# kaddly/GraphNeuralNetwork

Measured on NVIDIA B200. Metric: aggregated_edges_per_sec, higher is better.
Workload: dtype f32

## Files before the change

graphneuralnetwork_b200/_lib.py:

```python
from __future__ import annotations

import ctypes as C
import os
from pathlib import Path

_PKG = Path(__file__).resolve().parent
LIB_PATH = _PKG / "libgnn_b200.so"

i32, i64, f32, f64, u64 = C.c_int32, C.c_int64, C.c_float, C.c_double, C.c_uint64
ptr, size_t, cint = C.c_void_p, C.c_size_t, C.c_int

SIGNATURES = {
    "gnn_version": (cint, []),
    "gnn_last_error_string": (C.c_char_p, []),
    "gnn_status_string": (C.c_char_p, [cint]),
    "gnn_launch_count": (i64, []),
    "gnn_set_tuning": (cint, [C.c_char_p, cint]),
    "gnn_get_tuning": (cint, [C.c_char_p, C.POINTER(cint)]),
    "gnn_build_csr_from_coo_workspace_size": (size_t, [i64, i64]),
    "gnn_build_csr_from_coo": (cint, [ptr, ptr, ptr, i64, i64, i64, ptr, ptr, ptr, ptr, ptr, size_t, ptr]),
    "gnn_dense_mask_count_workspace_size": (size_t, [i64]),
    "gnn_dense_mask_count": (cint, [ptr, cint, i64, i64, i64, ptr, ptr, size_t, ptr]),
    "gnn_dense_mask_fill": (cint, [ptr, cint, i64, i64, i64, ptr, ptr, ptr]),
    "gnn_csr_transpose_workspace_size": (size_t, [i64, i64, i64]),
# ... 6 lines not shown
    "gnn_spmm_csr_planned_f32": (cint, [ptr, ptr, ptr, ptr, ptr, i64, i64, i32, i64, i64, ptr, i64, i64, ptr, i64, i32,
                                        cint, i32, ptr, i32, ptr, size_t, ptr]),
    "gnn_spmm_csr_planned_bf16": (cint, [ptr, ptr, ptr, ptr, ptr, i64, i64, i32, i64, i64, ptr, i64, i64, ptr, i64, i32,
                                         cint, i32, ptr, i32, ptr, size_t, ptr]),
    "gnn_sddmm_coo_f32": (cint, [ptr, ptr, cint, i64, ptr, i64, ptr, i64, i32, ptr, ptr]),
    "gnn_semantic_workspace_size": (i64, [i32]),
    "gnn_semantic_scores_f32": (cint, [ptr, i64, ptr, ptr, i64, i32, i32, ptr, ptr, ptr, i64, ptr]),
    "gnn_semantic_combine_f32": (cint, [ptr, ptr, i64, i32, i32, ptr, ptr]),
    "gnn_semantic_combine_bwd_f32": (cint, [ptr, ptr, ptr, i64, i32, i32, ptr, ptr, ptr, i64, ptr]),
    "gnn_semantic_scores_bwd_f32": (cint, [ptr, i64, ptr, ptr, ptr, i64, i32, i32, ptr, i64, ptr, ptr, ptr, i64, ptr]),
    "gnn_gather_reduce_f32": (cint, [ptr, i64, i64, ptr, cint, i64, i32, i32, cint, ptr, i64, ptr, ptr]),
    "gnn_gather_reduce_bf16": (cint, [ptr, i64, i64, ptr, cint, i64, i32, i32, cint, ptr, i64, ptr, ptr]),
    "gnn_gather_reduce_multi_f32": (cint, [ptr, i64, i64, i32, cint, i32, ptr, cint, ptr, ptr, ptr, ptr, ptr]),
    "gnn_gather_reduce_multi_bf16": (cint, [ptr, i64, i64, i32, cint, i32, ptr, cint, ptr, ptr, ptr, ptr, ptr]),
    "gnn_gather_reduce_multi_f32_split": (cint, [ptr, i64, i64, i32, cint, i32, ptr, cint, ptr, ptr, ptr, ptr, ptr, ptr]),
    "gnn_gather_reduce_typed_f32": (cint, [ptr, i64, i64, i32, ptr, cint, i64, i32, i32, cint, ptr, i64, ptr]),
    "gnn_gather_reduce_bwd_f32": (cint, [ptr, ptr, i64, i32, f32, ptr, i64, ptr, i64, i32, ptr]),
    "gnn_gather_reduce_bwd_dense_f32": (cint, [ptr, i64, ptr, i64, i32, i32, f32, ptr, ptr]),
    "gnn_sample_neighbors": (cint, [ptr, ptr, ptr, cint, i64, i32, u64, ptr, ptr, cint, ptr]),
    "gnn_gat_scores_f32": (cint, [ptr, i64, ptr, ptr, i64, i32, i32, ptr, ptr, ptr]),
    "gnn_gat_fused_fwd_f32": (cint, [ptr, ptr, ptr, i64, ptr, ptr, i64, i64, i32, i32, f32, cint, cint, ptr, ptr, ptr,
                                     i64, ptr, ptr, ptr, i64, i64, i64, ptr]),
    "gnn_gat_fused_bwd_f32": (cint, [ptr, ptr, ptr, ptr, ptr, ptr, i64, ptr, ptr, ptr, ptr, ptr, ptr, i64, i64, i32,
                                     i32, f32, cint, ptr, ptr, i64, ptr, ptr, ptr, i64, ptr, i64, ptr, i64, i64, cint,
                                     ptr, ptr, i64, ptr]),
    "gnn_gat_fused_fwd_train_f32": (cint, [ptr, ptr, ptr, i64, ptr, ptr, i64, i64, i32, i32, f32, cint, cint, ptr, ptr,
                                           ptr, ptr, ptr, i64, ptr, ptr, ptr, i64, i64, i64, ptr]),
    "gnn_gat_fused_fwd_train_bf16": (cint, [ptr, ptr, ptr, i64, ptr, ptr, i64, i64, i32, i32, f32, cint, cint, ptr, ptr,
                                            ptr, ptr, ptr, i64, ptr, ptr, ptr, i64, i64, i64, ptr]),
    "gnn_gat_fused_fwd_bf16": (cint, [ptr, ptr, ptr, i64, ptr, ptr, i64, i64, i32, i32, f32, cint, cint, ptr, ptr, ptr,
# ... 17 lines not shown
    "gnn_spmm_csr_ex_f32": (cint, [ptr, ptr, ptr, ptr, ptr, i64, i64, i32, i64, i64, ptr, ptr]),
    "gnn_spmm_csr_ex_bf16": (cint, [ptr, ptr, ptr, ptr, ptr, i64, i64, i32, i64, i64, ptr, ptr]),
}



class SpmmOpts(C.Structure):
    _fields_ = [("struct_size", i32), ("accumulate", i32), ("accumulate_prefix", i64), ("rows_per_team", i32),
                ("relu", i32), ("bias", ptr), ("row_map", ptr), ("X2", ptr), ("ldx2", i64), ("split", i64),
                ("long_rows", ptr), ("n_long", i64), ("long_threshold", i64), ("chunk_off", ptr), ("n_chunks", i64),
                ("chunk_edges", i32), ("exclusion_smem_bytes", i32), ("workspace", ptr), ("workspace_bytes", size_t)]


class GatDropout(C.Structure):
    _fields_ = [("struct_size", i32), ("p", f32), ("seed", u64), ("seed_dev", ptr)]


class HaloOpts(C.Structure):
    _fields_ = [("struct_size", i32), ("mover", i32), ("ctas", i32), ("warps_per_cta", i32),
                ("claim_smem_bytes", i32), ("first_peer", i32)]


GNN_OK = 0
REDUCE = {"mean": 0, "sum": 1, "max": 2}
GAT_SOFTMAX, GAT_EXPNEG = 0, 1

_lib = None


class GnnError(RuntimeError):
# ... 42 lines not shown
```

graphneuralnetwork_b200/csrc/api.cu:

```cuda
#include "common.cuh"
#include <string.h>
#include <mutex>
#include <map>
#include <string>

namespace gnn {

static thread_local char t_err[512] = "";
std::atomic<int64_t> g_launches{0};

void set_error(const char* fmt, ...) {
  va_list ap;
  va_start(ap, fmt);
  vsnprintf(t_err, sizeof(t_err), fmt, ap);
  va_end(ap);
}

int num_sms() {
  static int cache[64] = {0};
  int dev = 0;
  if (cudaGetDevice(&dev) != cudaSuccess || dev < 0 || dev >= 64) return 148;
  if (cache[dev] == 0) {
    int n = 0;
    if (cudaDeviceGetAttribute(&n, cudaDevAttrMultiProcessorCount, dev) != cudaSuccess || n <= 0) n = 148;
    cache[dev] = n;
  }
  return cache[dev];
}

static std::mutex g_tune_mu;
static std::map<std::string, int>& tune_map() {
  static std::map<std::string, int> m = {
      {"sage.smem_kb", 48},
      {"sage.chunk_bytes", 12288},
      {"sage.force_ldg", 0},
      {"sage.ctas_per_sm", 4},
      {"sage.packed_add", -1},
      {"spmm.long_row", 2048},
      {"spmm.chunk", 8192},
      {"spmm.unroll", 0},
      {"spmm.ctas3", 1},
      {"spmm.rows_per_team", 0},
      {"spmm.team_edges", 512},
      {"gat.stage_edges", 128},
      {"gat.bwd_stage_edges", 64},
      {"gat.coop_min_avg_deg", 256},
      {"gat.long_row", 1024},
  };
  return m;
}
int tuning(const char* key, int dflt) {
// ... 56 lines not shown
```

graphneuralnetwork_b200/csrc/sage.cu:

```cuda
#include "rowreduce.cuh"

using namespace gnn;

namespace {

constexpr int kConsumerWarps = 5;
constexpr int kConsumerThreads = kConsumerWarps * 32;
constexpr int kSageThreads = 32 + kConsumerThreads;
constexpr int kMaxBlocks = 4;
constexpr int kIdDepth = 4;

template <typename T>
struct SageArgs {
  const T* table;
  int64_t ld;
  int32_t F;
  int32_t n_blocks;
  const int32_t* idx32[kMaxBlocks];
  const int64_t* idx64[kMaxBlocks];
  int64_t src_off[kMaxBlocks + 1];
  int32_t fanout[kMaxBlocks];
  int32_t kc[kMaxBlocks];
  float scale[kMaxBlocks];
  T* out[kMaxBlocks];
  int64_t ldo[kMaxBlocks];
  int32_t* argmax[kMaxBlocks];
  int32_t out_vec16[kMaxBlocks];
  int32_t row_bytes;
  int32_t stage_rows;
  int32_t stages;
  int32_t nvec;
  int64_t n_table_rows;
  int32_t split[kMaxBlocks];
  int64_t lo_off[kMaxBlocks];
};

__device__ __forceinline__ void add2(float& a0, float& a1, float x0, float x1) {
  asm("{\n\t.reg .b64 ra, rx;\n\tmov.b64 ra, {%0, %1};\n\tmov.b64 rx, {%2, %3};\n\t"
      "add.rn.f32x2 ra, ra, rx;\n\tmov.b64 {%0, %1}, ra;\n\t}"
      : "+f"(a0), "+f"(a1)
      : "f"(x0), "f"(x1));
}

template <typename T>
struct Vec16;
template <>
struct Vec16<float> {
  static constexpr int E = 4;
  static __device__ __forceinline__ void unpack(const uint4& w, float (&o)[4]) {
// ... 31 lines not shown
  if (g < a.src_off[a.n_blocks]) {
    int b = 0;
    while (b + 1 < a.n_blocks && g >= a.src_off[b + 1]) ++b;
    c.b = b;
    c.src = g - a.src_off[b];
    c.fan = a.fanout[b];
    c.kc = a.kc[b];
  }
}
template <typename T>
__device__ __forceinline__ void cursor_next(Cursor& c, const SageArgs<T>& a) {
  c.c0 += c.kc;
  if (c.c0 >= c.fan) cursor_set(c, a, c.g + gridDim.x);
}

template <typename T, int NV, int OP, bool PK = true>
__global__ void __launch_bounds__(kSageThreads) sage_tma_kernel(const SageArgs<T> a) {
  constexpr int E = Vec16<T>::E;
  extern __shared__ __align__(128) unsigned char smem[];
  const int S = a.stages;
  const int stage_bytes = a.stage_rows * a.row_bytes;
  uint64_t* full = reinterpret_cast<uint64_t*>(smem + (size_t)S * stage_bytes);
  uint64_t* empty = full + S;
  uint32_t* mask = reinterpret_cast<uint32_t*>(empty + S);

  const int warp = threadIdx.x >> 5;
  const int lane = threadIdx.x & 31;
  if (threadIdx.x == 0) {
    for (int i = 0; i < S; ++i) {
      mbar_init(full + i, 1);
      mbar_init(empty + i, kConsumerWarps);
// ... 62 lines not shown
          best[v][i] = 0;
        }
    };
    reset();
    Cursor cur;
    cursor_set(cur, a, blockIdx.x);
    int stage = 0;
    uint32_t par = 0;
    for (; cur.g < total_src; cursor_next(cur, a)) {
      const int c0 = cur.c0;
      const int rows = min(cur.kc, cur.fan - c0);
      mbar_wait(full + stage, par);
      const unsigned m = mask[stage];
      const unsigned char* sb = smem + (size_t)stage * stage_bytes;
      const unsigned all_rows = rows >= 32 ? 0xffffffffu : ((1u << rows) - 1u);
      if (OP != GNN_REDUCE_MAX && m == all_rows) {
#pragma unroll 5
        for (int k = 0; k < rows; ++k) {
#pragma unroll
          for (int v = 0; v < NV; ++v) {
            const int vi = t + v * kConsumerThreads;
            if (vi < a.nvec) {
              const uint4 w = *reinterpret_cast<const uint4*>(sb + (size_t)k * a.row_bytes + (size_t)vi * 16);
              if (PK) {
                Vec16<T>::add(w, acc[v]);
              } else {
                float x[E];
                Vec16<T>::unpack(w, x);
#pragma unroll
                for (int i = 0; i < E; ++i) acc[v][i] += x[i];
              }
            }
          }
        }
      } else {
#pragma unroll 4
        for (int k = 0; k < rows; ++k) {
          if (!((m >> k) & 1u)) continue;
#pragma unroll
          for (int v = 0; v < NV; ++v) {
            const int vi = t + v * kConsumerThreads;
            if (vi < a.nvec) {
              const uint4 w = *reinterpret_cast<const uint4*>(sb + (size_t)k * a.row_bytes + (size_t)vi * 16);
              float x[E];
              Vec16<T>::unpack(w, x);
#pragma unroll
              for (int i = 0; i < E; ++i) {
                if (OP == GNN_REDUCE_MAX) {
                  if (x[i] > acc[v][i]) {
                    acc[v][i] = x[i];
                    best[v][i] = c0 + k;
                  }
                } else {
                  acc[v][i] += x[i];
                }
              }
            }
          }
        }
      }
// ... 49 lines not shown
              for (int i = 0; i < E; ++i)
                if (col0 + i < a.F) a.argmax[b][cur.src * a.ldo[b] + col0 + i] = best[v][i];
            }
          }
        }
        reset();
      }
      if (++stage == S) {
        stage = 0;
        par ^= 1u;
      }
    }
  }
}

template <typename T, int NV, int OP, bool PK>
int launch_tma_pk(const SageArgs<T>& a, size_t smem_bytes, int grid, cudaStream_t st) {
  static size_t configured[64] = {};
  int dev = 0;
  const bool cached = cudaGetDevice(&dev) == cudaSuccess && dev >= 0 && dev < 64;
  if (!cached || smem_bytes > configured[dev]) {
    GNN_CUDA(cudaFuncSetAttribute(sage_tma_kernel<T, NV, OP, PK>, cudaFuncAttributeMaxDynamicSharedMemorySize,
                                  (int)smem_bytes));
    if (cached) configured[dev] = smem_bytes;
  }
  sage_tma_kernel<T, NV, OP, PK><<<grid, kSageThreads, smem_bytes, st>>>(a);
  GNN_LAUNCH_CHECK();
  return GNN_OK;
}

template <typename T, int NV, int OP>
int launch_tma_inst(const SageArgs<T>& a, size_t smem_bytes, int grid, cudaStream_t st) {
  const int knob = tuning("sage.packed_add", -1);
  const bool pk = (OP != GNN_REDUCE_MAX) && (knob < 0 ? sizeof(T) == 2 : knob != 0);
  if (pk) return launch_tma_pk<T, NV, OP, true>(a, smem_bytes, grid, st);
  return launch_tma_pk<T, NV, OP, false>(a, smem_bytes, grid, st);
}

template <typename T, int OP>
int launch_tma(const SageArgs<T>& a, size_t smem_bytes, int grid, cudaStream_t st) {
  const int nv = (a.nvec + kConsumerThreads - 1) / kConsumerThreads;
  switch (nv) {
    case 1: return launch_tma_inst<T, 1, OP>(a, smem_bytes, grid, st);
    case 2: return launch_tma_inst<T, 2, OP>(a, smem_bytes, grid, st);
    case 3: return launch_tma_inst<T, 3, OP>(a, smem_bytes, grid, st);
    case 4: return launch_tma_inst<T, 4, OP>(a, smem_bytes, grid, st);
    default: break;
  }
  set_error("TMA gather: row too wide (nvec=%d)", a.nvec);
  return GNN_ERR_UNSUPPORTED;
}

template <typename T>
struct GatherBlock {
  const void* idx;
  int idx_bits;
  int64_t n_src;
  int32_t fanout;
  T* out;
  int64_t ldo;
  int32_t* argmax;
  int32_t split = 0;
  int64_t lo_off = 0;
};

template <typename T>
int gather_reduce_impl(const T* table, int64_t ld, int64_t n_table_rows, int32_t F, int reduce,
                       const GatherBlock<T>* blocks, int n_blocks, cudaStream_t st) {
  GNN_REQUIRE(F >= 0 && n_blocks >= 0 && n_blocks <= kMaxBlocks, GNN_ERR_BAD_ARG, "bad size (F=%d, blocks=%d, max %d)",
              F, n_blocks, kMaxBlocks);
  GNN_REQUIRE(reduce == GNN_REDUCE_MEAN || reduce == GNN_REDUCE_SUM || reduce == GNN_REDUCE_MAX, GNN_ERR_BAD_ARG,
              "unknown reduce %d (GraphSAGE_Pytorch/models/Aggregator.py:26 raises ValueError)", reduce);
  GNN_REQUIRE(n_table_rows < 0x7fffffffLL, GNN_ERR_UNSUPPORTED, "table rows do not fit int32");
  int64_t total_src = 0;
  for (int b = 0; b < n_blocks; ++b) {
    const GatherBlock<T>& k = blocks[b];
    GNN_REQUIRE(k.n_src >= 0 && k.fanout >= 0, GNN_ERR_BAD_ARG, "negative size");
    if (k.n_src == 0 || F == 0) continue;
    GNN_REQUIRE(k.fanout > 0, GNN_ERR_BAD_ARG, "fanout must be positive");
    GNN_REQUIRE(table && k.out, GNN_ERR_BAD_ARG, "null table/out");
    GNN_REQUIRE(k.idx == nullptr || k.idx_bits == 32 || k.idx_bits == 64, GNN_ERR_BAD_ARG, "idx_bits must be 32 or 64");
    GNN_REQUIRE(ld >= F && k.ldo >= F, GNN_ERR_BAD_ARG, "leading dimension smaller than F");
    GNN_REQUIRE(!k.split || (sizeof(T) == 4 && reduce != GNN_REDUCE_MAX && k.lo_off >= F && k.ldo % 4 == 0 &&
                             k.lo_off % 4 == 0 && aligned_to(k.out, 8)),
                GNN_ERR_BAD_ARG, "hi/lo fp16 output needs an fp32 table, mean/sum, 8-byte aligned planes");
    GNN_REQUIRE(k.idx != nullptr || k.n_src * (int64_t)k.fanout <= n_table_rows, GNN_ERR_BAD_ARG,
                "identity block needs n_src*fanout <= n_table_rows");
    total_src += k.n_src;
  }
  if (total_src == 0 || F == 0) return GNN_OK;

  const int esz = (int)sizeof(T);
  const int row_bytes = (int)round_up((size_t)F * esz, 16);
  const bool tma_ok = !tuning("sage.force_ldg", 0) && aligned_to(table, 16) && ((ld * esz) % 16 == 0) &&
                      (int64_t)row_bytes <= ld * esz && row_bytes >= 256 && (row_bytes / 16) <= 4 * kConsumerThreads;
  if (tma_ok) {
    SageArgs<T> a{};
    a.table = table;
    a.ld = ld;
    a.F = F;
    a.n_table_rows = n_table_rows;
    a.row_bytes = row_bytes;
    a.nvec = row_bytes / 16;
    const int E = 16 / esz;
    int kc0 = tuning("sage.chunk_bytes", 12288) / row_bytes;
    kc0 = kc0 < 1 ? 1 : kc0;
    kc0 = kc0 > 32 ? 32 : kc0;
    const size_t budget = (size_t)tuning("sage.smem_kb", 48) * 1024;
// ... 6 lines not shown
      a.idx32[nb] = (k.idx && k.idx_bits == 32) ? (const int32_t*)k.idx : nullptr;
      a.idx64[nb] = (k.idx && k.idx_bits == 64) ? (const int64_t*)k.idx : nullptr;
      a.fanout[nb] = k.fanout;
      int kc = kc0 > k.fanout ? k.fanout : kc0;
      const int nchunk = (k.fanout + kc - 1) / kc;
      kc = (k.fanout + nchunk - 1) / nchunk;
      a.kc[nb] = kc;
      stage_rows = kc > stage_rows ? kc : stage_rows;
      a.scale[nb] = (reduce == GNN_REDUCE_MEAN) ? 1.0f / (float)k.fanout : 1.0f;
      a.out[nb] = k.out;
      a.ldo[nb] = k.ldo;
      a.argmax[nb] = (reduce == GNN_REDUCE_MAX) ? k.argmax : nullptr;
      a.out_vec16[nb] = aligned_to(k.out, 16) && ((k.ldo * esz) % 16 == 0) && ((int64_t)a.nvec * E <= k.ldo);
      a.split[nb] = k.split;
      a.lo_off[nb] = k.lo_off;
      a.src_off[nb + 1] = a.src_off[nb] + k.n_src;
      ++nb;
    }
    a.n_blocks = nb;
    a.stage_rows = stage_rows;
    int stages = (int)(budget / ((size_t)stage_rows * row_bytes));
    stages = stages > 8 ? 8 : stages;
    GNN_REQUIRE(stages >= 2, GNN_ERR_UNSUPPORTED, "row of %d bytes does not fit the shared-memory ring", row_bytes);
    a.stages = stages;
    const size_t smem_bytes = (size_t)stages * stage_rows * row_bytes + (size_t)stages * (16 + 4) + 16;
    int64_t grid = (int64_t)num_sms() * tuning("sage.ctas_per_sm", 4);
    grid = grid > total_src ? total_src : grid;
    switch (reduce) {
      case GNN_REDUCE_MAX: return launch_tma<T, GNN_REDUCE_MAX>(a, smem_bytes, (int)grid, st);
      default: return launch_tma<T, GNN_REDUCE_SUM>(a, smem_bytes, (int)grid, st);
// ... 11 lines not shown
    r.fanout = k.fanout;
    r.col32 = (k.idx && k.idx_bits == 32) ? (const int32_t*)k.idx : nullptr;
    r.col64 = (k.idx && k.idx_bits == 64) ? (const int64_t*)k.idx : nullptr;
    r.val = nullptr;
    r.src_div = 0;
    r.scale = (reduce == GNN_REDUCE_MEAN) ? 1.0f / (float)k.fanout : 1.0f;
    r.n_src_rows = (int32_t)n_table_rows;
    r.X = table;
    r.ldx = ld;
    r.Y = k.out;
    r.ldy = k.ldo;
    r.n_rows = k.n_src;
    r.F = F;
    r.skip_deg_gt = 0;
    r.argmax = (reduce == GNN_REDUCE_MAX) ? k.argmax : nullptr;
    const int rc = (reduce == GNN_REDUCE_MAX) ? launch_row_reduce<T, 1>(r, st) : launch_row_reduce<T, 0>(r, st);
    if (rc != GNN_OK) return rc;
  }
  return GNN_OK;
}

template <typename T>
int gather_reduce_multi(const T* table, int64_t ld, int64_t n_table_rows, int32_t F, int reduce, int32_t n_blocks,
                        const void* const* idx, int idx_bits, const int64_t* n_src, const int32_t* fanout,
                        void* const* out, const int64_t* ld_out, cudaStream_t st) {
  GNN_REQUIRE(n_blocks >= 0 && n_blocks <= kMaxBlocks, GNN_ERR_UNSUPPORTED, "at most %d blocks per launch", kMaxBlocks);
  GNN_REQUIRE(n_blocks == 0 || (idx && n_src && fanout && out && ld_out), GNN_ERR_BAD_ARG, "null block array");
  GatherBlock<T> blocks[kMaxBlocks];
  for (int b = 0; b < n_blocks; ++b)
    blocks[b] = GatherBlock<T>{idx[b], idx_bits, n_src[b], fanout[b], (T*)out[b], ld_out[b], nullptr};
  return gather_reduce_impl<T>(table, ld, n_table_rows, F, reduce, blocks, n_blocks, st);
}
// ... 43 lines not shown
}

int gnn_gather_reduce_multi_f32_split(const float* table, int64_t ld_table, int64_t n_table_rows, int32_t F, int reduce,
                                      int32_t n_blocks, const void* const* idx_host, int idx_bits,
                                      const int64_t* n_src_host, const int32_t* fanout_host, void* const* out_hi_host,
                                      const int64_t* ld_out_host, const int64_t* lo_off_host, gnn_stream_t stream) {
  GNN_REQUIRE(n_blocks >= 0 && n_blocks <= kMaxBlocks, GNN_ERR_UNSUPPORTED, "at most %d blocks per launch", kMaxBlocks);
  GNN_REQUIRE(n_blocks == 0 || (idx_host && n_src_host && fanout_host && out_hi_host && ld_out_host && lo_off_host),
              GNN_ERR_BAD_ARG, "null block array");
  GatherBlock<float> blocks[kMaxBlocks];
  for (int b = 0; b < n_blocks; ++b) {
    blocks[b] = GatherBlock<float>{idx_host[b], idx_bits, n_src_host[b], fanout_host[b], (float*)out_hi_host[b],
                                   ld_out_host[b], nullptr};
    blocks[b].split = 1;
    blocks[b].lo_off = lo_off_host[b];
  }
  return gather_reduce_impl<float>(table, ld_table, n_table_rows, F, reduce, blocks, n_blocks, (cudaStream_t)stream);
}

int gnn_gather_reduce_multi_bf16(const void* table, int64_t ld_table, int64_t n_table_rows, int32_t F, int reduce,
                                 int32_t n_blocks, const void* const* idx_host, int idx_bits,
                                 const int64_t* n_src_host, const int32_t* fanout_host, void* const* out_host,
                                 const int64_t* ld_out_host, gnn_stream_t stream) {
  return gather_reduce_multi<__nv_bfloat16>((const __nv_bfloat16*)table, ld_table, n_table_rows, F, reduce, n_blocks,
                                            idx_host, idx_bits, n_src_host, fanout_host, out_host, ld_out_host,
                                            (cudaStream_t)stream);
}

int gnn_gather_reduce_typed_f32(const float* table, int64_t ld_row, int64_t n_nodes, int32_t n_types, const void* idx,
                                int idx_bits, int64_t n_src, int32_t fanout, int32_t F, int reduce, float* out,
// ... 74 lines not shown
```

graphneuralnetwork_b200/functional.py:

```python
from __future__ import annotations

from typing import Optional

import torch

from . import _lib
from .graph import CSRGraph, _p, _require_cuda, _stream_ptr, index_block_transpose


def _rowmajor(x: torch.Tensor) -> torch.Tensor:
    if x.dim() != 2:
        raise _lib.GnnError(f"expected a 2-D feature matrix, got shape {tuple(x.shape)}")
    if x.stride(1) != 1 and x.shape[1] > 1:
        x = x.contiguous()
    if x.shape[0] > 1 and x.stride(0) < x.shape[1]:
        x = x.contiguous()
    return x


def _ld(x: torch.Tensor) -> int:
    return x.stride(0) if x.shape[0] > 1 else max(x.shape[1], 1)


def _padded_empty(rows: int, F: int, dtype, device) -> torch.Tensor:
# ... 258 lines not shown
        if idx.numel() != n_src * fanout:
            raise _lib.GnnError(f"index block has {idx.numel()} ids, expected n_src*fanout = {n_src * fanout}")
        idxs.append(idx)
    for o in outs_hi:
        if o.dtype != torch.float16 or o.stride(1) != 1:
            raise _lib.GnnError("gather_reduce_multi_split: outputs must be fp16 views with unit column stride")
    idx_arr = (C.c_void_p * nb)(*[_p(i) for i in idxs])
    nsrc_arr = (C.c_int64 * nb)(*[int(b[1]) for b in blocks])
    fan_arr = (C.c_int32 * nb)(*[int(b[2]) for b in blocks])
    out_arr = (C.c_void_p * nb)(*[_p(o) for o in outs_hi])
    ldo_arr = (C.c_int64 * nb)(*[_ld(o) for o in outs_hi])
    lo_arr = (C.c_int64 * nb)(*[int(lo_off)] * nb)
    _lib.check(lib.gnn_gather_reduce_multi_f32_split(_p(table), _ld(table), N, F, _lib.REDUCE[reduce], nb, idx_arr,
                                                     bits or 64, nsrc_arr, fan_arr, out_arr, ldo_arr, lo_arr,
                                                     _stream_ptr()), "gnn_gather_reduce_multi_f32_split")


def sample_neighbors(g: CSRGraph, src: torch.Tensor, k: int, seed: int, out_dtype=torch.int32,
                     seed_offset: Optional[torch.Tensor] = None, out: Optional[torch.Tensor] = None) -> torch.Tensor:
    _require_cuda(src)
    lib = _lib.load()
    src = src.contiguous().view(-1)
    if src.dtype not in (torch.int32, torch.int64):
        src = src.to(torch.int64)
    if out is None:
        out = torch.empty(src.numel() * k, dtype=out_dtype, device=src.device)
    assert seed_offset is None or (seed_offset.dtype == torch.int64 and seed_offset.is_cuda)
    _lib.check(lib.gnn_sample_neighbors(_p(g.rowptr), _p(g.col), _p(src), 32 if src.dtype == torch.int32 else 64,
                                        src.numel(), int(k), int(seed) & 0xFFFFFFFFFFFFFFFF, _p(seed_offset), _p(out),
                                        32 if out.dtype == torch.int32 else 64, _stream_ptr()), "gnn_sample_neighbors")
# ... 433 lines not shown
```

graphneuralnetwork_b200/layers/sage.py:

```python
import torch
from torch import nn
import torch.nn.functional as F

from .. import _lib
from ..functional import gather_reduce, gather_reduce_multi_raw, gather_reduce_multi_split_raw, pad_table


class SampledBlock:

    def __init__(self, table: torch.Tensor, ids: torch.Tensor, fanout: int):
        self.table, self.ids, self.fanout = table, ids, int(fanout)
        self.n_src = ids.numel() // self.fanout


class NeighborAggregator(nn.Module):

    def __init__(self, input_dim, output_dim, use_bias=False, aggr_method="mean", **kwargs):
        super().__init__(**kwargs)
        self.input_dim, self.output_dim = input_dim, output_dim
        self.use_bias, self.aggr_method = use_bias, aggr_method
        self.weight = nn.Parameter(nn.init.xavier_uniform_(torch.empty(input_dim, output_dim)))
        if use_bias:
            self.bias = nn.Parameter(torch.zeros(output_dim))

# ... 100 lines not shown
        if getattr(self, "tensor_core_gemm", True) and layer0.aggr_neighbor_method in ("mean", "sum") \
                and table.stride(0) * 4 % 16 == 0 and F_in * 4 >= 256:
            try:
                return self._layer0_split_gemm(table, node_id_blocks, ld, n_hop, total)
            except _lib.GnnError:
                self.tensor_core_gemm = False
        key = (total, table.device)
        buf = getattr(self, "_l0_buf", None)
        if buf is None or buf[0] != key:
            Z = torch.zeros((total, 2 * ld), dtype=torch.float32, device=table.device)
            Wc = torch.zeros((2 * ld, H), dtype=torch.float32, device=table.device)
            self._l0_buf = buf = (key, Z, Wc)
        _, Z, Wc = buf
        Wc[:F_in].copy_(layer0.weight)
        Wc[ld:ld + F_in].copy_(layer0.aggregator.weight)
        blocks, outs, row = [], [], 0
        for hop in range(L):
            n = n_hop[hop]
            blocks += [(node_id_blocks[hop + 1], n, fan[hop]), (node_id_blocks[hop], n, 1)]
            outs += [Z[row:row + n, ld:ld + F_in], Z[row:row + n, :F_in]]
            row += n
        order = sorted(range(len(blocks)), key=lambda i: -blocks[i][1] * blocks[i][2])
        gather_reduce_multi_raw(table, [blocks[i] for i in order], layer0.aggr_neighbor_method,
                                outs=[outs[i] for i in order])
        hidden = torch.mm(Z, Wc)
        if layer0.activation:
            hidden = layer0.activation(hidden)
        out, row = [], 0
        for n in n_hop:
            out.append(hidden[row:row + n])
            row += n
        return out

    def _table_fits_fp16(self, table):
        key = (table.data_ptr(), table._version, tuple(table.shape))
        hit = getattr(self, "_fp16_ok", None)
        if hit is None or hit[0] != key:
            self._fp16_ok = hit = (key, bool((table.abs().max() < 3.0e4).item()))
        return hit[1]

    def _weight_planes(self, ld, device):
        layer0 = self.gcn[0]
        w, wa = layer0.weight, layer0.aggregator.weight
        F_in, H = layer0.input_dim, layer0.hidden_dim
        geom = (int(ld), torch.device(device))
        ver = (w._version, wa._version, w.data_ptr(), wa.data_ptr())
        planes = getattr(self, "_l0_planes", None)
# ... 13 lines not shown
            planes["ver"] = ver
        return planes["hi"], planes["lo"]

    def _layer0_split_gemm(self, table, node_id_blocks, ld, n_hop, total):
        if not self._table_fits_fp16(table):
            raise _lib.GnnError("table exceeds the fp16 range: fp32 product")
        L, fan, layer0 = self.num_layers, self.num_neighbors_list, self.gcn[0]
        F_in, H = layer0.input_dim, layer0.hidden_dim
        key = (total, table.device)
        buf = getattr(self, "_l0_split", None)
        if buf is None or buf[0] != key:
            Zs = torch.zeros((total, 4 * ld), dtype=torch.float16, device=table.device)
            self._l0_split = buf = (key, Zs)
        _, Zs = buf
        W_hi, W_lo = self._weight_planes(ld, table.device)
        blocks, outs, row = [], [], 0
        for hop in range(L):
            n = n_hop[hop]
            blocks += [(node_id_blocks[hop + 1], n, fan[hop]), (node_id_blocks[hop], n, 1)]
            outs += [Zs[row:row + n, ld:ld + F_in], Zs[row:row + n, :F_in]]
            row += n
        order = sorted(range(len(blocks)), key=lambda i: -blocks[i][1] * blocks[i][2])
        gather_reduce_multi_split_raw(table, [blocks[i] for i in order], layer0.aggr_neighbor_method,
                                      [outs[i] for i in order], lo_off=2 * ld)
        Z_hi, Z_lo = Zs[:, :2 * ld], Zs[:, 2 * ld:]
        hidden = torch.mm(Z_hi, W_hi, out_dtype=torch.float32)
        if getattr(self, "_addmm_out_dtype", True):
            try:
                hidden = torch.addmm(hidden, Z_lo, W_hi, out_dtype=torch.float32)
                hidden = torch.addmm(hidden, Z_hi, W_lo, out_dtype=torch.float32)
            except (RuntimeError, NotImplementedError):
                self._addmm_out_dtype = False
                hidden = torch.mm(Z_hi, W_hi, out_dtype=torch.float32)
        if not getattr(self, "_addmm_out_dtype", True):
            hidden += torch.mm(Z_lo, W_hi, out_dtype=torch.float32)
            hidden += torch.mm(Z_hi, W_lo, out_dtype=torch.float32)
        if layer0.activation:
            hidden = layer0.activation(hidden)
        out, row = [], 0
# ... 117 lines not shown
```

include/gnn_b200.h:

```cpp
#ifndef GNN_B200_H
#define GNN_B200_H

#include <stddef.h>
#include <stdint.h>

#ifdef __cplusplus
extern "C" {
#endif

typedef void* gnn_stream_t;

typedef enum {
  GNN_OK = 0,
  GNN_ERR_BAD_ARG = 1,
  GNN_ERR_MISALIGNED = 2,
  GNN_ERR_UNSUPPORTED = 3,
  GNN_ERR_CUDA = 4,
  GNN_ERR_WORKSPACE = 5
} gnn_status;

typedef enum { GNN_REDUCE_MEAN = 0, GNN_REDUCE_SUM = 1, GNN_REDUCE_MAX = 2 } gnn_reduce;

typedef enum {
  GNN_GAT_SOFTMAX = 0,
// ... 97 lines not shown
                           const void* idx, int idx_bits, int64_t n_src, int32_t fanout, int32_t F,
                           int reduce, void* out, int64_t ld_out, int32_t* argmax, gnn_stream_t stream);
int gnn_gather_reduce_multi_f32(const float* table, int64_t ld_table, int64_t n_table_rows, int32_t F, int reduce,
                                int32_t n_blocks, const void* const* idx_host, int idx_bits,
                                const int64_t* n_src_host, const int32_t* fanout_host,
                                void* const* out_host, const int64_t* ld_out_host, gnn_stream_t stream);
int gnn_gather_reduce_multi_bf16(const void* table, int64_t ld_table, int64_t n_table_rows, int32_t F, int reduce,
                                 int32_t n_blocks, const void* const* idx_host, int idx_bits,
                                 const int64_t* n_src_host, const int32_t* fanout_host,
                                 void* const* out_host, const int64_t* ld_out_host, gnn_stream_t stream);
int gnn_gather_reduce_multi_f32_split(const float* table, int64_t ld_table, int64_t n_table_rows, int32_t F, int reduce,
                                      int32_t n_blocks, const void* const* idx_host, int idx_bits,
                                      const int64_t* n_src_host, const int32_t* fanout_host,
                                      void* const* out_hi_host, const int64_t* ld_out_host,
                                      const int64_t* lo_off_host, gnn_stream_t stream);
int gnn_gather_reduce_typed_f32(const float* table, int64_t ld_row, int64_t n_nodes, int32_t n_types,
                                const void* idx, int idx_bits, int64_t n_src, int32_t fanout, int32_t F,
                                int reduce, float* out, int64_t ld_out, gnn_stream_t stream);
int gnn_gather_reduce_bwd_f32(const int64_t* rowptr_t, const int32_t* pos_t, int64_t n_table_rows,
                              int32_t fanout, float scale, const float* d_out, int64_t ld_dout,
                              float* d_table, int64_t ld_dtable, int32_t F, gnn_stream_t stream);
int gnn_gather_reduce_bwd_dense_f32(const float* d_out, int64_t ld_dout, const int32_t* argmax ,
                                    int64_t n_src, int32_t fanout, int32_t F, float scale,
                                    float* d_neigh , gnn_stream_t stream);

int gnn_sample_neighbors(const int64_t* rowptr, const int32_t* col, const void* src, int src_bits,
                         int64_t n_src, int32_t k, uint64_t seed, const int64_t* seed_offset_dev,
                         void* out, int out_bits, gnn_stream_t stream);

int gnn_gat_scores_f32(const float* Wh, int64_t ldw, const float* a_src, const float* a_dst,
// ... 131 lines not shown
```

Baseline: 2.022 billion.

## Echo gathered neighbor rows as next hop's self features; add narrow-row cp.async gather

In the layer-0 SAGE gather, the neighbor rows already staged for hop h are written out as the self-feature rows of hop h+1. This replaces the separate fanout-1 self gathers for all hops except the first, so those table rows are not read from global memory a second time. A separate cp.async warp-per-source kernel is added for fp32 mean/sum with rows of at most 512 bytes, used when split and echo are off. The echo path adds stores inside the TMA consumer loop and more template variants, and the narrow path bypasses the TMA pipeline for small F.

After: 2.062 billion, median of 6. 2.0% higher.

```diff
diff --git a/graphneuralnetwork_b200/_lib.py b/graphneuralnetwork_b200/_lib.py
--- a/graphneuralnetwork_b200/_lib.py
+++ b/graphneuralnetwork_b200/_lib.py
@@ -44,6 +44,7 @@
     "gnn_gather_reduce_multi_f32": (cint, [ptr, i64, i64, i32, cint, i32, ptr, cint, ptr, ptr, ptr, ptr, ptr]),
     "gnn_gather_reduce_multi_bf16": (cint, [ptr, i64, i64, i32, cint, i32, ptr, cint, ptr, ptr, ptr, ptr, ptr]),
     "gnn_gather_reduce_multi_f32_split": (cint, [ptr, i64, i64, i32, cint, i32, ptr, cint, ptr, ptr, ptr, ptr, ptr, ptr]),
+    "gnn_gather_reduce_multi_f32_ex": (cint, [ptr, i64, i64, i32, cint, i32, ptr, ptr]),
     "gnn_gather_reduce_typed_f32": (cint, [ptr, i64, i64, i32, ptr, cint, i64, i32, i32, cint, ptr, i64, ptr]),
     "gnn_gather_reduce_bwd_f32": (cint, [ptr, ptr, i64, i32, f32, ptr, i64, ptr, i64, i32, ptr]),
     "gnn_gather_reduce_bwd_dense_f32": (cint, [ptr, i64, ptr, i64, i32, i32, f32, ptr, ptr]),
@@ -91,6 +92,11 @@
 
 class GatDropout(C.Structure):
     _fields_ = [("struct_size", i32), ("p", f32), ("seed", u64), ("seed_dev", ptr)]
+
+
+class GatherBlock(C.Structure):
+    _fields_ = [("struct_size", i32), ("idx_bits", i32), ("idx", ptr), ("n_src", i64), ("fanout", i32), ("split", i32),
+                ("out", ptr), ("ld_out", i64), ("lo_off", i64), ("echo", ptr), ("ld_echo", i64)]
 
 
 class HaloOpts(C.Structure):
diff --git a/graphneuralnetwork_b200/csrc/api.cu b/graphneuralnetwork_b200/csrc/api.cu
--- a/graphneuralnetwork_b200/csrc/api.cu
+++ b/graphneuralnetwork_b200/csrc/api.cu
@@ -35,6 +35,7 @@
       {"sage.chunk_bytes", 12288},
       {"sage.force_ldg", 0},
       {"sage.ctas_per_sm", 4},
+      {"sage.narrow_ldg", -1},
       {"sage.packed_add", -1},
       {"spmm.long_row", 2048},
       {"spmm.chunk", 8192},
diff --git a/graphneuralnetwork_b200/csrc/sage.cu b/graphneuralnetwork_b200/csrc/sage.cu
--- a/graphneuralnetwork_b200/csrc/sage.cu
+++ b/graphneuralnetwork_b200/csrc/sage.cu
@@ -33,6 +33,9 @@
   int64_t n_table_rows;
   int32_t split[kMaxBlocks];
   int64_t lo_off[kMaxBlocks];
+  void* echo[kMaxBlocks];
+  int64_t ld_echo[kMaxBlocks];
+  int32_t echo_vec16[kMaxBlocks];
 };
 
 __device__ __forceinline__ void add2(float& a0, float& a1, float x0, float x1) {
@@ -94,7 +97,48 @@
   if (c.c0 >= c.fan) cursor_set(c, a, c.g + gridDim.x);
 }
 
-template <typename T, int NV, int OP, bool PK = true>
+template <typename T, int E>
+__device__ __forceinline__ void store_vec(void* out, int64_t ld, int64_t row, int col0, int F, int split,
+                                          int64_t lo_off, int vec16, const float (&o)[E]) {
+  if (sizeof(T) == 4 && split) {
+    __half* hrow = reinterpret_cast<__half*>(out) + row * ld + col0;
+    uint32_t hw[2], lw[2];
+#pragma unroll
+    for (int i = 0; i < 2; ++i) {
+      const __half h0 = __float2half_rn(o[2 * i]), h1 = __float2half_rn(o[2 * i + 1]);
+      const __half l0 = __float2half_rn(o[2 * i] - __half2float(h0));
+      const __half l1 = __float2half_rn(o[2 * i + 1] - __half2float(h1));
+      hw[i] = (uint32_t)__half_as_ushort(h0) | ((uint32_t)__half_as_ushort(h1) << 16);
+      lw[i] = (uint32_t)__half_as_ushort(l0) | ((uint32_t)__half_as_ushort(l1) << 16);
+    }
+    if (col0 + 3 < F) {
+      *reinterpret_cast<uint2*>(hrow) = make_uint2(hw[0], hw[1]);
+      *reinterpret_cast<uint2*>(hrow + lo_off) = make_uint2(lw[0], lw[1]);
+    } else {
+#pragma unroll
+      for (int i = 0; i < 4; ++i)
+        if (col0 + i < F) {
+          const __half h = __float2half_rn(o[i]);
+          hrow[i] = h;
+          hrow[lo_off + i] = __float2half_rn(o[i] - __half2float(h));
+        }
+    }
+  } else {
+    T* orow = reinterpret_cast<T*>(out) + row * ld + col0;
+    if (vec16) {
+      VecIO<T, E>::store(orow, o);
+    } else {
+#pragma unroll
+      for (int i = 0; i < E; ++i)
+        if (col0 + i < F) {
+          float o1[1] = {o[i]};
+          VecIO<T, 1>::store(orow + i, o1);
+        }
+    }
+  }
+}
+
+template <typename T, int NV, int OP, bool PK, bool ECHO>
 __global__ void __launch_bounds__(kSageThreads) sage_tma_kernel(const SageArgs<T> a) {
   constexpr int E = Vec16<T>::E;
   extern __shared__ __align__(128) unsigned char smem[];
@@ -187,6 +231,15 @@
       const unsigned m = mask[stage];
       const unsigned char* sb = smem + (size_t)stage * stage_bytes;
       const unsigned all_rows = rows >= 32 ? 0xffffffffu : ((1u << rows) - 1u);
+      void* const echo = ECHO ? a.echo[cur.b] : nullptr;
+      const int64_t erow0 = cur.src * cur.fan + c0;
+      auto echo_vec = [&](int k, int vi, const float (&x)[E]) {
+        float o[E];
+#pragma unroll
+        for (int i = 0; i < E; ++i) o[i] = x[i] + 0.f;
+        store_vec<T, E>(echo, a.ld_echo[cur.b], erow0 + k, vi * E, a.F, a.split[cur.b], a.lo_off[cur.b],
+                        a.echo_vec16[cur.b], o);
+      };
       if (OP != GNN_REDUCE_MAX && m == all_rows) {
 #pragma unroll 5
         for (int k = 0; k < rows; ++k) {
@@ -203,20 +256,32 @@
 #pragma unroll
                 for (int i = 0; i < E; ++i) acc[v][i] += x[i];
               }
+              if (ECHO && echo) {
+                float x[E];
+                Vec16<T>::unpack(w, x);
+                echo_vec(k, vi, x);
+              }
             }
           }
         }
       } else {
 #pragma unroll 4
         for (int k = 0; k < rows; ++k) {
-          if (!((m >> k) & 1u)) continue;
+          const bool valid = (m >> k) & 1u;
+          if (!valid && !(ECHO && echo)) continue;
 #pragma unroll
           for (int v = 0; v < NV; ++v) {
             const int vi = t + v * kConsumerThreads;
             if (vi < a.nvec) {
-              const uint4 w = *reinterpret_cast<const uint4*>(sb + (size_t)k * a.row_bytes + (size_t)vi * 16);
               float x[E];
-              Vec16<T>::unpack(w, x);
+              if (valid) {
+                Vec16<T>::unpack(*reinterpret_cast<const uint4*>(sb + (size_t)k * a.row_bytes + (size_t)vi * 16), x);
+              } else {
+#pragma unroll
+                for (int i = 0; i < E; ++i) x[i] = 0.f;
+              }
+              if (ECHO && echo) echo_vec(k, vi, x);
+              if (!valid) continue;
 #pragma unroll
               for (int i = 0; i < E; ++i) {
                 if (OP == GNN_REDUCE_MAX) {
@@ -296,17 +361,17 @@
   }
 }
 
-template <typename T, int NV, int OP, bool PK>
+template <typename T, int NV, int OP, bool PK, bool ECHO>
 int launch_tma_pk(const SageArgs<T>& a, size_t smem_bytes, int grid, cudaStream_t st) {
   static size_t configured[64] = {};
   int dev = 0;
   const bool cached = cudaGetDevice(&dev) == cudaSuccess && dev >= 0 && dev < 64;
   if (!cached || smem_bytes > configured[dev]) {
-    GNN_CUDA(cudaFuncSetAttribute(sage_tma_kernel<T, NV, OP, PK>, cudaFuncAttributeMaxDynamicSharedMemorySize,
+    GNN_CUDA(cudaFuncSetAttribute(sage_tma_kernel<T, NV, OP, PK, ECHO>, cudaFuncAttributeMaxDynamicSharedMemorySize,
                                   (int)smem_bytes));
     if (cached) configured[dev] = smem_bytes;
   }
-  sage_tma_kernel<T, NV, OP, PK><<<grid, kSageThreads, smem_bytes, st>>>(a);
+  sage_tma_kernel<T, NV, OP, PK, ECHO><<<grid, kSageThreads, smem_bytes, st>>>(a);
   GNN_LAUNCH_CHECK();
   return GNN_OK;
 }
@@ -315,8 +380,18 @@
 int launch_tma_inst(const SageArgs<T>& a, size_t smem_bytes, int grid, cudaStream_t st) {
   const int knob = tuning("sage.packed_add", -1);
   const bool pk = (OP != GNN_REDUCE_MAX) && (knob < 0 ? sizeof(T) == 2 : knob != 0);
-  if (pk) return launch_tma_pk<T, NV, OP, true>(a, smem_bytes, grid, st);
-  return launch_tma_pk<T, NV, OP, false>(a, smem_bytes, grid, st);
+  bool echo = false;
+  for (int b = 0; b < a.n_blocks; ++b) echo = echo || a.echo[b] != nullptr;
+  if (echo) {
+    if constexpr (sizeof(T) == 4 && OP != GNN_REDUCE_MAX) {
+      if (pk) return launch_tma_pk<T, NV, OP, true, true>(a, smem_bytes, grid, st);
+      return launch_tma_pk<T, NV, OP, false, true>(a, smem_bytes, grid, st);
+    }
+    set_error("echo rows: fp32 mean/sum only");
+    return GNN_ERR_UNSUPPORTED;
+  }
+  if (pk) return launch_tma_pk<T, NV, OP, true, false>(a, smem_bytes, grid, st);
+  return launch_tma_pk<T, NV, OP, false, false>(a, smem_bytes, grid, st);
 }
 
 template <typename T, int OP>
@@ -331,6 +406,56 @@
   }
   set_error("TMA gather: row too wide (nvec=%d)", a.nvec);
   return GNN_ERR_UNSUPPORTED;
+}
+
+constexpr int kNarrowChunk = 32;
+constexpr int kNarrowWarps = 2;
+
+__global__ void __launch_bounds__(kNarrowWarps * 32) sage_narrow_kernel(
+    const float* __restrict__ table, int64_t ld, int64_t n_table_rows, const int32_t* __restrict__ idx32,
+    const int64_t* __restrict__ idx64, int64_t n_src, int fanout, int chunk, int nvec, int F, float scale, float* out,
+    int64_t ldo, int out_vec16) {
+  extern __shared__ __align__(16) float4 stage[];
+  const int lane = threadIdx.x & 31;
+  const int64_t src = (int64_t)blockIdx.x * kNarrowWarps + (threadIdx.x >> 5);
+  if (src >= n_src) return;
+  float4* mine = stage + (size_t)(threadIdx.x >> 5) * chunk * 32 + lane;
+  const bool active = lane < nvec;
+  float acc[4] = {0.f, 0.f, 0.f, 0.f};
+  for (int c0 = 0; c0 < fanout; c0 += chunk) {
+    int64_t my = -1;
+    if (lane < chunk && c0 + lane < fanout) {
+      const int64_t p = src * fanout + c0 + lane;
+      my = idx32 ? (int64_t)__ldg(idx32 + p) : idx64 ? __ldg(idx64 + p) : p;
+    }
+    const unsigned ok = __ballot_sync(0xffffffffu, my >= 0 && my < n_table_rows);
+    for (int k = 0; k < chunk; ++k) {
+      const int64_t r = __shfl_sync(0xffffffffu, my, k);
+      if (active && ((ok >> k) & 1u)) {
+        const uint32_t dst = (uint32_t)__cvta_generic_to_shared(mine + k * 32);
+        asm volatile("cp.async.cg.shared.global [%0], [%1], 16;\n" ::"r"(dst), "l"(table + r * ld + lane * 4));
+      }
+    }
+    asm volatile("cp.async.commit_group;\ncp.async.wait_group 0;\n" ::: "memory");
+    if (active) {
+      const int n = min(chunk, fanout - c0);
+      for (int k = 0; k < n; ++k) {
+        if ((ok >> k) & 1u) {
+          const float4 x = mine[k * 32];
+          acc[0] += x.x;
+          acc[1] += x.y;
+          acc[2] += x.z;
+          acc[3] += x.w;
+        }
+      }
+    }
+    __syncwarp();
+  }
+  if (!active) return;
+  float o[4];
+#pragma unroll
+  for (int i = 0; i < 4; ++i) o[i] = acc[i] * scale;
+  store_vec<float, 4>(out, ldo, src, lane * 4, F, 0, 0, out_vec16, o);
 }
 
 template <typename T>
@@ -344,6 +469,8 @@
   int32_t* argmax;
   int32_t split = 0;
   int64_t lo_off = 0;
+  void* echo = nullptr;
+  int64_t ld_echo = 0;
 };
 
 template <typename T>
@@ -368,12 +495,35 @@
                 GNN_ERR_BAD_ARG, "hi/lo fp16 output needs an fp32 table, mean/sum, 8-byte aligned planes");
     GNN_REQUIRE(k.idx != nullptr || k.n_src * (int64_t)k.fanout <= n_table_rows, GNN_ERR_BAD_ARG,
                 "identity block needs n_src*fanout <= n_table_rows");
+    GNN_REQUIRE(!k.echo || (reduce != GNN_REDUCE_MAX && k.ld_echo >= F &&
+                            (!k.split || (k.ld_echo % 4 == 0 && aligned_to(k.echo, 8)))),
+                GNN_ERR_BAD_ARG, "echo rows need mean/sum, ld_echo >= F (split: 8-byte aligned planes)");
     total_src += k.n_src;
   }
   if (total_src == 0 || F == 0) return GNN_OK;
 
   const int esz = (int)sizeof(T);
   const int row_bytes = (int)round_up((size_t)F * esz, 16);
+  const int narrow_knob = tuning("sage.narrow_ldg", -1);
+  bool narrow = narrow_knob != 0 && !tuning("sage.force_ldg", 0) && esz == 4 && row_bytes <= 512 &&
+                reduce != GNN_REDUCE_MAX && aligned_to(table, 16) && ((ld * esz) % 16 == 0);
+  for (int b = 0; b < n_blocks; ++b) narrow = narrow && !blocks[b].split && !blocks[b].echo;
+  if (narrow) {
+    for (int b = 0; b < n_blocks; ++b) {
+      const GatherBlock<T>& k = blocks[b];
+      if (k.n_src == 0) continue;
+      const int64_t grid = (k.n_src + kNarrowWarps - 1) / kNarrowWarps;
+      GNN_REQUIRE(grid < 0x7fffffffLL, GNN_ERR_UNSUPPORTED, "too many sources for one grid: %lld", (long long)k.n_src);
+      const int vec16 = aligned_to(k.out, 16) && ((k.ldo * esz) % 16 == 0) && ((int64_t)(row_bytes / 4) <= k.ldo);
+      const int chunk = k.fanout < kNarrowChunk ? k.fanout : kNarrowChunk;
+      sage_narrow_kernel<<<(unsigned)grid, kNarrowWarps * 32, (size_t)kNarrowWarps * chunk * 32 * 16, st>>>(
+          (const float*)table, ld, n_table_rows, (k.idx && k.idx_bits == 32) ? (const int32_t*)k.idx : nullptr,
+          (k.idx && k.idx_bits == 64) ? (const int64_t*)k.idx : nullptr, k.n_src, k.fanout, chunk, row_bytes / 16, F,
+          (reduce == GNN_REDUCE_MEAN) ? 1.0f / (float)k.fanout : 1.0f, (float*)k.out, k.ldo, vec16);
+      GNN_LAUNCH_CHECK();
+    }
+    return GNN_OK;
+  }
   const bool tma_ok = !tuning("sage.force_ldg", 0) && aligned_to(table, 16) && ((ld * esz) % 16 == 0) &&
                       (int64_t)row_bytes <= ld * esz && row_bytes >= 256 && (row_bytes / 16) <= 4 * kConsumerThreads;
   if (tma_ok) {
@@ -410,6 +560,9 @@
       a.out_vec16[nb] = aligned_to(k.out, 16) && ((k.ldo * esz) % 16 == 0) && ((int64_t)a.nvec * E <= k.ldo);
       a.split[nb] = k.split;
       a.lo_off[nb] = k.lo_off;
+      a.echo[nb] = k.echo;
+      a.ld_echo[nb] = k.ld_echo;
+      a.echo_vec16[nb] = aligned_to(k.echo, 16) && ((k.ld_echo * esz) % 16 == 0) && ((int64_t)a.nvec * E <= k.ld_echo);
       a.src_off[nb + 1] = a.src_off[nb] + k.n_src;
       ++nb;
     }
@@ -451,8 +604,17 @@
     r.F = F;
     r.skip_deg_gt = 0;
     r.argmax = (reduce == GNN_REDUCE_MAX) ? k.argmax : nullptr;
-    const int rc = (reduce == GNN_REDUCE_MAX) ? launch_row_reduce<T, 1>(r, st) : launch_row_reduce<T, 0>(r, st);
+    int rc = (reduce == GNN_REDUCE_MAX) ? launch_row_reduce<T, 1>(r, st) : launch_row_reduce<T, 0>(r, st);
     if (rc != GNN_OK) return rc;
+    if (k.echo) {
+      r.fanout = 1;
+      r.scale = 1.0f;
+      r.Y = (T*)k.echo;
+      r.ldy = k.ld_echo;
+      r.n_rows = k.n_src * (int64_t)k.fanout;
+      rc = launch_row_reduce<T, 0>(r, st);
+      if (rc != GNN_OK) return rc;
+    }
   }
   return GNN_OK;
 }
@@ -526,6 +688,24 @@
                                    ld_out_host[b], nullptr};
     blocks[b].split = 1;
     blocks[b].lo_off = lo_off_host[b];
+  }
+  return gather_reduce_impl<float>(table, ld_table, n_table_rows, F, reduce, blocks, n_blocks, (cudaStream_t)stream);
+}
+
+int gnn_gather_reduce_multi_f32_ex(const float* table, int64_t ld_table, int64_t n_table_rows, int32_t F, int reduce,
+                                   int32_t n_blocks, const gnn_gather_block* blocks_host, gnn_stream_t stream) {
+  GNN_REQUIRE(n_blocks >= 0 && n_blocks <= kMaxBlocks, GNN_ERR_UNSUPPORTED, "at most %d blocks per launch", kMaxBlocks);
+  GNN_REQUIRE(n_blocks == 0 || blocks_host, GNN_ERR_BAD_ARG, "null block array");
+  GatherBlock<float> blocks[kMaxBlocks];
+  for (int b = 0; b < n_blocks; ++b) {
+    const gnn_gather_block& k = blocks_host[b];
+    GNN_REQUIRE(k.struct_size == (int32_t)sizeof(gnn_gather_block), GNN_ERR_BAD_ARG,
+                "gnn_gather_block.struct_size is %d, expected %d", k.struct_size, (int)sizeof(gnn_gather_block));
+    blocks[b] = GatherBlock<float>{k.idx, k.idx_bits, k.n_src, k.fanout, (float*)k.out, k.ld_out, nullptr};
+    blocks[b].split = k.split;
+    blocks[b].lo_off = k.lo_off;
+    blocks[b].echo = k.echo;
+    blocks[b].ld_echo = k.ld_echo;
   }
   return gather_reduce_impl<float>(table, ld_table, n_table_rows, F, reduce, blocks, n_blocks, (cudaStream_t)stream);
 }
diff --git a/graphneuralnetwork_b200/functional.py b/graphneuralnetwork_b200/functional.py
--- a/graphneuralnetwork_b200/functional.py
+++ b/graphneuralnetwork_b200/functional.py
@@ -296,6 +296,46 @@
     _lib.check(lib.gnn_gather_reduce_multi_f32_split(_p(table), _ld(table), N, F, _lib.REDUCE[reduce], nb, idx_arr,
                                                      bits or 64, nsrc_arr, fan_arr, out_arr, ldo_arr, lo_arr,
                                                      _stream_ptr()), "gnn_gather_reduce_multi_f32_split")
+
+
+def gather_reduce_multi_ex(table: torch.Tensor, blocks, reduce: str, outs, echos=None, lo_off: Optional[int] = None):
+    import ctypes as C
+    if reduce not in _lib.REDUCE:
+        raise ValueError("Unknown aggr type, expected sum, max, or mean, but got {}".format(reduce))
+    echos = list(echos) if echos is not None else [None] * len(blocks)
+    _require_cuda(table, *[b[0] for b in blocks], *outs, *[e for e in echos if e is not None])
+    lib = _lib.load()
+    table = _rowmajor(table)
+    if table.dtype != torch.float32:
+        raise _lib.GnnError("gather_reduce_multi_ex: fp32 table only")
+    if len(outs) != len(blocks) or len(echos) != len(blocks):
+        raise _lib.GnnError("gather_reduce_multi_ex: one output (and one echo entry) per block")
+    N, F = table.shape
+    odt = torch.float32 if lo_off is None else torch.float16
+    arr = (_lib.GatherBlock * max(len(blocks), 1))()
+    keep = []
+    for b, ((idx, n_src, fanout), out, echo) in enumerate(zip(blocks, outs, echos)):
+        if idx is not None:
+            idx = idx.contiguous().view(-1)
+            if idx.dtype not in (torch.int32, torch.int64):
+                idx = idx.to(torch.int64)
+            if idx.numel() != n_src * fanout:
+                raise _lib.GnnError(f"index block has {idx.numel()} ids, expected n_src*fanout = {n_src * fanout}")
+            keep.append(idx)
+        for t, rows in ((out, n_src), (echo, n_src * fanout)):
+            if t is not None and (t.dtype != odt or t.stride(1) != 1 or t.shape[0] != rows or t.shape[1] != F):
+                raise _lib.GnnError(f"gather_reduce_multi_ex: expected a [{rows}, {F}] {odt} view with unit column "
+                                    f"stride, got {tuple(t.shape)} {t.dtype}")
+        e = arr[b]
+        e.struct_size = C.sizeof(_lib.GatherBlock)
+        e.idx_bits = 32 if (idx is not None and idx.dtype == torch.int32) else 64
+        e.idx, e.n_src, e.fanout = _p(idx), int(n_src), int(fanout)
+        e.split, e.lo_off = (0, 0) if lo_off is None else (1, int(lo_off))
+        e.out, e.ld_out = _p(out), _ld(out)
+        e.echo, e.ld_echo = _p(echo), (_ld(echo) if echo is not None else 0)
+    _lib.check(lib.gnn_gather_reduce_multi_f32_ex(_p(table), _ld(table), N, F, _lib.REDUCE[reduce], len(blocks), arr,
+                                                  _stream_ptr()), "gnn_gather_reduce_multi_f32_ex")
+    return outs
 
 
 def sample_neighbors(g: CSRGraph, src: torch.Tensor, k: int, seed: int, out_dtype=torch.int32,
diff --git a/graphneuralnetwork_b200/layers/sage.py b/graphneuralnetwork_b200/layers/sage.py
--- a/graphneuralnetwork_b200/layers/sage.py
+++ b/graphneuralnetwork_b200/layers/sage.py
@@ -3,7 +3,7 @@
 import torch.nn.functional as F
 
 from .. import _lib
-from ..functional import gather_reduce, gather_reduce_multi_raw, gather_reduce_multi_split_raw, pad_table
+from ..functional import gather_reduce, gather_reduce_multi_ex, gather_reduce_multi_raw, pad_table
 
 
 class SampledBlock:
@@ -138,15 +138,7 @@
         _, Z, Wc = buf
         Wc[:F_in].copy_(layer0.weight)
         Wc[ld:ld + F_in].copy_(layer0.aggregator.weight)
-        blocks, outs, row = [], [], 0
-        for hop in range(L):
-            n = n_hop[hop]
-            blocks += [(node_id_blocks[hop + 1], n, fan[hop]), (node_id_blocks[hop], n, 1)]
-            outs += [Z[row:row + n, ld:ld + F_in], Z[row:row + n, :F_in]]
-            row += n
-        order = sorted(range(len(blocks)), key=lambda i: -blocks[i][1] * blocks[i][2])
-        gather_reduce_multi_raw(table, [blocks[i] for i in order], layer0.aggr_neighbor_method,
-                                outs=[outs[i] for i in order])
+        self._layer0_gather(table, node_id_blocks, n_hop, lambda r0, n, c: Z[r0:r0 + n, c:c + F_in], ld, None)
         hidden = torch.mm(Z, Wc)
         if layer0.activation:
             hidden = layer0.activation(hidden)
@@ -155,6 +147,24 @@
             out.append(hidden[row:row + n])
             row += n
         return out
+
+    def _layer0_gather(self, table, node_id_blocks, n_hop, view, ld, lo_off):
+        L, fan, layer0 = self.num_layers, self.num_neighbors_list, self.gcn[0]
+        starts = [sum(n_hop[:h]) for h in range(L)]
+        blocks, outs, echos = [], [], []
+        echo = getattr(self, "echo_self_rows", True)
+        for hop in range(L):
+            n, r0 = n_hop[hop], starts[hop]
+            blocks.append((node_id_blocks[hop + 1], n, fan[hop]))
+            outs.append(view(r0, n, ld))
+            echos.append(view(starts[hop + 1], n_hop[hop + 1], 0) if echo and hop + 1 < L else None)
+        for hop in (range(1) if echo else range(L)):
+            blocks.append((node_id_blocks[hop], n_hop[hop], 1))
+            outs.append(view(starts[hop], n_hop[hop], 0))
+            echos.append(None)
+        order = sorted(range(len(blocks)), key=lambda i: -blocks[i][1] * blocks[i][2])
+        gather_reduce_multi_ex(table, [blocks[i] for i in order], layer0.aggr_neighbor_method,
+                               [outs[i] for i in order], echos=[echos[i] for i in order], lo_off=lo_off)
 
     def _table_fits_fp16(self, table):
         key = (table.data_ptr(), table._version, tuple(table.shape))
@@ -198,15 +208,7 @@
             self._l0_split = buf = (key, Zs)
         _, Zs = buf
         W_hi, W_lo = self._weight_planes(ld, table.device)
-        blocks, outs, row = [], [], 0
-        for hop in range(L):
-            n = n_hop[hop]
-            blocks += [(node_id_blocks[hop + 1], n, fan[hop]), (node_id_blocks[hop], n, 1)]
-            outs += [Zs[row:row + n, ld:ld + F_in], Zs[row:row + n, :F_in]]
-            row += n
-        order = sorted(range(len(blocks)), key=lambda i: -blocks[i][1] * blocks[i][2])
-        gather_reduce_multi_split_raw(table, [blocks[i] for i in order], layer0.aggr_neighbor_method,
-                                      [outs[i] for i in order], lo_off=2 * ld)
+        self._layer0_gather(table, node_id_blocks, n_hop, lambda r0, n, c: Zs[r0:r0 + n, c:c + F_in], ld, 2 * ld)
         Z_hi, Z_lo = Zs[:, :2 * ld], Zs[:, 2 * ld:]
         hidden = torch.mm(Z_hi, W_hi, out_dtype=torch.float32)
         if getattr(self, "_addmm_out_dtype", True):
diff --git a/include/gnn_b200.h b/include/gnn_b200.h
--- a/include/gnn_b200.h
+++ b/include/gnn_b200.h
@@ -135,6 +135,21 @@
                                       const int64_t* n_src_host, const int32_t* fanout_host,
                                       void* const* out_hi_host, const int64_t* ld_out_host,
                                       const int64_t* lo_off_host, gnn_stream_t stream);
+typedef struct gnn_gather_block {
+  int32_t struct_size;
+  int32_t idx_bits;
+  const void* idx;
+  int64_t n_src;
+  int32_t fanout;
+  int32_t split;
+  void* out;
+  int64_t ld_out;
+  int64_t lo_off;
+  void* echo;
+  int64_t ld_echo;
+} gnn_gather_block;
+int gnn_gather_reduce_multi_f32_ex(const float* table, int64_t ld_table, int64_t n_table_rows, int32_t F, int reduce,
+                                   int32_t n_blocks, const gnn_gather_block* blocks_host, gnn_stream_t stream);
 int gnn_gather_reduce_typed_f32(const float* table, int64_t ld_row, int64_t n_nodes, int32_t n_types,
                                 const void* idx, int idx_bits, int64_t n_src, int32_t fanout, int32_t F,
                                 int reduce, float* out, int64_t ld_out, gnn_stream_t stream);
```
